# templeblock/llzlab

Hardware: AMD Instinct MI355X
Metric: Msamples/s/GPU (float32 FIR 257-tap, 4096 ch) + achieved HBM GB/s vs peak (higher is better)
Workload: dtype f32; 1 GPU; 4096-ch float32 FIR, 257 taps (llz_fir_lpf_cof 0.1 KAISER), 1048576 samples/ch per GPU, overlap-save-1024, channels sharded over 1 GPU(s); channels_per_gpu=4096, samples_per_channel=1048576, taps=257, algorithm=overlap-save-1024

## Files before the change

### llzlab_amd/csrc/kernels/fir_bank.hip

```cpp
#include "common.hpp"
#include "fft32.hpp"
#include "ols_walk.hpp"

namespace {

constexpr int BANK_BINS = LLZS_BANK_BINS;
constexpr int BANK_PITCH = LLZS_BANK_PITCH;
constexpr int BANK_IMG = 514;
constexpr size_t BANK_LDS_COMMON = 1024 * sizeof(float2) + (size_t)OLS_WAVES * 2 * OLS_XBUF * sizeof(float);

__device__ __forceinline__ void bank_filter(cf (&v)[32], cf (&u)[32], float *buf, const float2 *s_tw, const float2 *h, int l5,
                                            int col)
{
    ols_forward(v, buf, s_tw, l5, col);
    const float2 *up = h + l5, *dn = h - l5;
#pragma unroll
    for (int r = 0; r < 32; r++) {
        const int b = brev5(r);
        if (b < 16) {
            const float2 w = up[32 * b];
            u[b] = cmul<false>(v[r], cf{w.x, w.y});
        } else {
            const float2 w = dn[1024 - 32 * b];
            u[b] = cmul<true>(v[r], cf{w.x, w.y});
        }
    }
    ols_inverse(u, buf, s_tw, l5, col);
}

template <bool GLOBAL_H>
__global__ void __launch_bounds__(OLS_THREADS, 2)
k_fir_bank_ols_f32(const float *__restrict__ in, float *__restrict__ out, const float *__restrict__ hist,
                   const float2 *__restrict__ hbank , const float2 *__restrict__ twid, ols_geom G)
{
    extern __shared__ __attribute__((aligned(16))) char smem[];
    float2 *s_tw = reinterpret_cast<float2 *>(smem);
    for (int i = threadIdx.x; i < 1024; i += OLS_THREADS) s_tw[i] = twid[i];
    __syncthreads();
    const int lane = threadIdx.x & 63;
    const int wave = __builtin_amdgcn_readfirstlane(threadIdx.x >> 6);
    const int l5 = lane & 31;
    const ols_lane g = ols_lane_of(lane);
    const int slot = (threadIdx.x >> 6) * 2 + g.half;
    float *buf = reinterpret_cast<float *>(s_tw + 1024) + slot * OLS_XBUF;
    float2 *img = reinterpret_cast<float2 *>(smem + BANK_LDS_COMMON) + slot * BANK_IMG;
    const long halves_total = (long)gridDim.x * OLS_WAVES * 2;
    const long first = ((long)blockIdx.x * OLS_WAVES + wave) * 2;

    ols_seg cur[2] = {ols_locate(first, G), ols_locate(first + 1, G)};
    float halo[8];
    ols_raw raw;
    {
        const float *const row[2] = {in + (size_t)cur[0].c * G.in_pitch, in + (size_t)cur[1].c * G.in_pitch};
        const ols_seg own = g.half ? cur[1] : cur[0];
        ols_load_halo(halo, g.half ? row[1] : row[0], hist ? hist + (size_t)own.c * G.keep : nullptr, own.j0 * OLS_JOB,
                      g.col, G.keep, own.live);
        const int s0[2] = {cur[0].j0 * OLS_JOB, cur[1].j0 * OLS_JOB};
        const bool lv[2] = {cur[0].count > 0, cur[1].count > 0};
        ols_load(raw, row, s0, lv, g, G.n);
    }
    for (long sp = first; sp < G.total_segs; sp += halves_total) {
        const ols_seg nxt[2] = {ols_locate(sp + halves_total, G), ols_locate(sp + halves_total + 1, G)};
        const float *const row[2] = {in + (size_t)cur[0].c * G.in_pitch, in + (size_t)cur[1].c * G.in_pitch};
        float *const orow[2] = {out + (size_t)cur[0].c * G.out_pitch, out + (size_t)cur[1].c * G.out_pitch};
        const float *const nrow[2] = {in + (size_t)nxt[0].c * G.in_pitch, in + (size_t)nxt[1].c * G.in_pitch};
        const ols_seg nown = g.half ? nxt[1] : nxt[0];
        float halo_n[8];
#pragma unroll
        for (int i = 0; i < 8; i++) halo_n[i] = 0.f;

        const ols_seg own = g.half ? cur[1] : cur[0];
        const float2 *hrow = hbank + (size_t)own.c * BANK_PITCH;
        if (!GLOBAL_H && own.live) {
#pragma unroll
            for (int i = 0; i < 16; i++) img[l5 + 32 * i] = hrow[l5 + 32 * i];
            if (l5 == 0) img[BANK_BINS - 1] = hrow[BANK_BINS - 1];
        }
        const float2 *h = GLOBAL_H ? hrow : img;

        const int jmax = max(cur[0].count, cur[1].count);
#pragma unroll 1
        for (int jj = 0; jj < jmax; jj++) {
            const int s[2] = {(cur[0].j0 + jj) * OLS_JOB, (cur[1].j0 + jj) * OLS_JOB};
            const bool live[2] = {jj < cur[0].count, jj < cur[1].count};
            cf v[32], u[32];
            ols_assemble(v, halo, raw);
            const bool in_pair = jj + 1 < jmax;
            {
                const float *const lrow[2] = {in_pair ? row[0] : nrow[0], in_pair ? row[1] : nrow[1]};
                const int sn[2] = {in_pair ? s[0] + OLS_JOB : nxt[0].j0 * OLS_JOB,
                                   in_pair ? s[1] + OLS_JOB : nxt[1].j0 * OLS_JOB};
                const bool ln[2] = {in_pair ? jj + 1 < cur[0].count : nxt[0].count > 0,
                                    in_pair ? jj + 1 < cur[1].count : nxt[1].count > 0};
                ols_load(raw, lrow, sn, ln, g, G.n);
            }
            if (!in_pair)
                ols_load_halo(halo_n, g.half ? nrow[1] : nrow[0], hist ? hist + (size_t)nown.c * G.keep : nullptr,
                              nown.j0 * OLS_JOB, g.col, G.keep, nown.live);
            bank_filter(v, u, buf, s_tw, h, l5, g.col);
            ols_store(u, orow, s, live, g, G.n);
        }
        cur[0] = nxt[0];
        cur[1] = nxt[1];
#pragma unroll
        for (int i = 0; i < 8; i++) halo[i] = halo_n[i];
    }
}

const ols_rung BANK_RUNGS[2] = {
    {1024, 1, "k_fir_bank_ols_f32", OLS_THREADS, 2 * OLS_WAVES, 2, true, 1.0,
     BANK_LDS_COMMON + (size_t)OLS_WAVES * 2 * BANK_IMG * sizeof(float2), false, false,
     1, {OLS_HALO}, {kfn(k_fir_bank_ols_f32<false>)}},
    {1024, 1, "k_fir_bank_ols_f32<global>", OLS_THREADS, 2 * OLS_WAVES, 2, true, 1.0,
     BANK_LDS_COMMON, false, false,
     1, {OLS_HALO}, {kfn(k_fir_bank_ols_f32<true>)}},
};

}

extern "C" int llzs_fir_bank_ols_f32(const float *hbank, const float *twid, const float *in, float *out, const float *hist,
                                     int channels, int n, long in_pitch, long out_pitch, int flt_len, void *stream)
{
    if (!hbank || !twid || !in || !out || channels <= 0 || n <= 0 || in_pitch < n || out_pitch < n) {
        llzs_set_error("fir_bank_ols_f32: bad arguments");
        return LLZ_ERR_ARG;
    }
    if (flt_len < 1 || flt_len - 1 > OLS_HALO) {
        llzs_set_error("fir_bank_ols_f32: flt_len %d outside 1..%d", flt_len, OLS_HALO + 1);
        return LLZ_ERR_RANGE;
    }
    const ols_rung &r = BANK_RUNGS[llzs_tune(LLZS_TUNE_BANK_GLOBAL_H) == 1 ? 1 : 0];
    ols_plan p = ols_plan_of(r, channels, n, in_pitch, out_pitch, flt_len);
    const float2 *hf = reinterpret_cast<const float2 *>(hbank), *tw = reinterpret_cast<const float2 *>(twid);
    void *args[6] = {&in, &out, &hist, &hf, &tw, &p.G};
    const void *kernel = r.kernel[0];
    if (r.lds_bytes > 64 * 1024)
        LLZ_HIP_CHECK(hipFuncSetAttribute(kernel, hipFuncAttributeMaxDynamicSharedMemorySize, (int)r.lds_bytes));
    (void)hipLaunchKernel(kernel, dim3((unsigned)p.blocks), dim3(r.threads), args, r.lds_bytes, as_stream(stream));
    LLZ_LAUNCH_CHECK(r.name);
    return LLZ_OK;
}
```

### llzlab_amd/csrc/kernels/fir_ols.hip

```cpp
#include <stdlib.h>
#include "common.hpp"
#include "fft32.hpp"
#include "ols_walk.hpp"

namespace {

constexpr int OLS_OVERLAP = 256;
static_assert(OLS_OVERLAP == OLS_HALO, "ols_walk.hpp carries the same overlap");

struct ols_smem {
    float2 *tw, *h;
    float *buf;
};

__device__ __forceinline__ ols_smem ols_tables(char *smem, const float2 *__restrict__ hfreq, const float2 *__restrict__ twid)
{
    ols_smem m;
    m.tw = reinterpret_cast<float2 *>(smem);
    m.h = m.tw + 1024;
    for (int i = threadIdx.x; i < 1024; i += OLS_THREADS) {
        m.tw[i] = twid[i];
        m.h[i] = hfreq[i];
    }
    __syncthreads();
    const int wave = threadIdx.x >> 6, half = (threadIdx.x >> 5) & 1;
    m.buf = reinterpret_cast<float *>(m.h + 1024) + (wave * 2 + half) * OLS_XBUF;
    return m;
}

__global__ void __launch_bounds__(OLS_THREADS, 2)
k_fir_ols_chain_f32(const float *__restrict__ in, float *__restrict__ out, const float *__restrict__ hist,
                    const float2 *__restrict__ hfreq, const float2 *__restrict__ twid, ols_geom G)
{
    extern __shared__ __attribute__((aligned(16))) char smem[];
    const ols_smem S = ols_tables(smem, hfreq, twid);
    const int lane = threadIdx.x & 63;
    const int wave = __builtin_amdgcn_readfirstlane(threadIdx.x >> 6);
    const int l5 = lane & 31;
    const ols_lane g = ols_lane_of(lane);
    const long halves_total = (long)gridDim.x * OLS_WAVES * 2;
    const long first = ((long)blockIdx.x * OLS_WAVES + wave) * 2;

    ols_seg cur[2] = {ols_locate(first, G), ols_locate(first + 1, G)};
    float halo[8];
    ols_raw raw;
    {
        const float *const row[2] = {in + (size_t)cur[0].c * G.in_pitch, in + (size_t)cur[1].c * G.in_pitch};
        const ols_seg own = g.half ? cur[1] : cur[0];
        ols_load_halo(halo, g.half ? row[1] : row[0], hist ? hist + (size_t)own.c * G.keep : nullptr, own.j0 * OLS_JOB,
                      g.col, G.keep, own.live);
        const int s0[2] = {cur[0].j0 * OLS_JOB, cur[1].j0 * OLS_JOB};
        const bool lv[2] = {cur[0].count > 0, cur[1].count > 0};
        ols_load(raw, row, s0, lv, g, G.n);
    }
    for (long sp = first; sp < G.total_segs; sp += halves_total) {
        const ols_seg nxt[2] = {ols_locate(sp + halves_total, G), ols_locate(sp + halves_total + 1, G)};
        const float *const row[2] = {in + (size_t)cur[0].c * G.in_pitch, in + (size_t)cur[1].c * G.in_pitch};
        float *const orow[2] = {out + (size_t)cur[0].c * G.out_pitch, out + (size_t)cur[1].c * G.out_pitch};
        const float *const nrow[2] = {in + (size_t)nxt[0].c * G.in_pitch, in + (size_t)nxt[1].c * G.in_pitch};
        const ols_seg nown = g.half ? nxt[1] : nxt[0];
        float halo_n[8];
#pragma unroll
        for (int i = 0; i < 8; i++) halo_n[i] = 0.f;

        const int jmax = max(cur[0].count, cur[1].count);
#pragma unroll 1
        for (int jj = 0; jj < jmax; jj++) {
            const int s[2] = {(cur[0].j0 + jj) * OLS_JOB, (cur[1].j0 + jj) * OLS_JOB};
            const bool live[2] = {jj < cur[0].count, jj < cur[1].count};
            cf v[32], u[32];
            ols_assemble(v, halo, raw);
            const bool in_pair = jj + 1 < jmax;
            {
                const float *const lrow[2] = {in_pair ? row[0] : nrow[0], in_pair ? row[1] : nrow[1]};
                const int sn[2] = {in_pair ? s[0] + OLS_JOB : nxt[0].j0 * OLS_JOB,
                                   in_pair ? s[1] + OLS_JOB : nxt[1].j0 * OLS_JOB};
                const bool ln[2] = {in_pair ? jj + 1 < cur[0].count : nxt[0].count > 0,
                                    in_pair ? jj + 1 < cur[1].count : nxt[1].count > 0};
                ols_load(raw, lrow, sn, ln, g, G.n);
            }
            if (!in_pair)
                ols_load_halo(halo_n, g.half ? nrow[1] : nrow[0], hist ? hist + (size_t)nown.c * G.keep : nullptr,
                              nown.j0 * OLS_JOB, g.col, G.keep, nown.live);
            ols_filter(v, u, S.buf, S.tw, S.h, l5, g.col);
            ols_store(u, orow, s, live, g, G.n);
        }
        cur[0] = nxt[0];
        cur[1] = nxt[1];
#pragma unroll
        for (int i = 0; i < 8; i++) halo[i] = halo_n[i];
    }
}



template <int O>
__global__ void __launch_bounds__(OLS_THREADS, 2)
k_fir_ols2k_chain_f32(const float *__restrict__ in, float *__restrict__ out, const float *__restrict__ hist,
                     const float2 *__restrict__ hfreq2 ,
                     const float2 *__restrict__ twid , const float2 *__restrict__ tw2k ,
                     ols_geom G)
{
    extern __shared__ __attribute__((aligned(16))) char smem[];
    float2 *s_tw = reinterpret_cast<float2 *>(smem);
    float2 *s_h = s_tw + 1024;
    float2 *s_w = s_h + 2048;
    for (int i = threadIdx.x; i < 1024; i += OLS_THREADS) {
        s_tw[i] = twid[i];
        s_h[i] = hfreq2[i];
        s_h[1024 + i] = hfreq2[1024 + i];
        s_w[i] = tw2k[i];
    }
    __syncthreads();
    constexpr int O2K_OVERLAP = O, O2K_VALID = 2048 - O, O2K_JOB = 2 * O2K_VALID;
    constexpr int HP = O / 64, NEW = 32 - HP;
    const int lane = threadIdx.x & 63;
    const int wave = __builtin_amdgcn_readfirstlane(threadIdx.x >> 6);
    const int half = lane >> 5, l5 = lane & 31;
    float *buf = reinterpret_cast<float *>(s_w + 1024) + (wave * 2 + half) * OLS_XBUF;
    const float2 *my_h = s_h + half * 1024;
    const long waves_total = (long)gridDim.x * OLS_WAVES;
    const int rowoff = 32 * half + l5;

    struct segd { const float *row; float *orow; const float *hrow; int j0, count; };
    auto locate = [&](long seg) {
        segd d;
        const bool live = seg < G.total_segs;
        const int c = live ? (int)(seg / G.segs_per_channel) : 0;
        d.j0 = live ? (int)(seg - (long)c * G.segs_per_channel) * G.seg_len : 0;
        d.count = live ? min(G.seg_len, G.jobs_per_channel - d.j0) : 0;
        d.row = in + (size_t)c * G.in_pitch;
        d.orow = out + (size_t)c * G.out_pitch;
        d.hrow = hist ? hist + (size_t)c * G.keep : nullptr;
        return d;
    };
    const int n = G.n;
    auto load_halo = [&](float (&halo)[HP], const segd &d) {
#pragma unroll
        for (int i = 0; i < HP; i++) {
            const int idx = d.j0 * O2K_JOB - O2K_OVERLAP + 64 * i + rowoff;
            float v = 0.f;
            if (d.count > 0) {
                if (idx >= 0) v = d.row[idx];
                else if (d.hrow && idx >= -G.keep) v = d.hrow[G.keep + idx];
            }
            halo[i] = v;
        }
    };
    ols_raw raw;
    auto load = [&](const float *row, int s, bool live) {
        if (live && s + O2K_JOB <= n) {
#pragma unroll
            for (int i = 0; i < NEW; i++) {
                raw.a[i] = __builtin_nontemporal_load(&row[s + 64 * i + rowoff]);
                raw.b[i] = __builtin_nontemporal_load(&row[s + O2K_VALID + 64 * i + rowoff]);
            }
        } else {
#pragma unroll
            for (int i = 0; i < NEW; i++) {
                const int ia = s + 64 * i + rowoff, ib = ia + O2K_VALID;
                const float xa = row[min(ia, n - 1)], xb = row[min(ib, n - 1)];
                raw.a[i] = (live && ia < n) ? xa : 0.f;
                raw.b[i] = (live && ib < n) ? xb : 0.f;
            }
        }
    };

    long seg = (long)blockIdx.x * OLS_WAVES + wave;
    segd cur = locate(seg);
    float halo[HP];
    load_halo(halo, cur);
    load(cur.row, cur.j0 * O2K_JOB, cur.count > 0);
    for (; seg < G.total_segs; seg += waves_total) {
        const segd nxt = locate(seg + waves_total);
        float halo_n[HP];
#pragma unroll
        for (int i = 0; i < HP; i++) halo_n[i] = 0.f;
#pragma unroll 1
        for (int jj = 0; jj < cur.count; jj++) {
            const int s = (cur.j0 + jj) * O2K_JOB;
            const float *row = cur.row;
            float *orow = cur.orow;
            cf v[32], u[32];
#pragma unroll
            for (int i = 0; i < HP; i++) {
                v[i].x = halo[i];
                v[i].y = raw.a[NEW - HP + i];
                halo[i] = raw.b[NEW - HP + i];
            }
#pragma unroll
            for (int i = 0; i < NEW; i++) {
                v[HP + i].x = raw.a[i];
                v[HP + i].y = raw.b[i];
            }
            const bool in_seg = jj + 1 < cur.count;
            load(in_seg ? row : nxt.row, in_seg ? s + O2K_JOB : nxt.j0 * O2K_JOB, in_seg || nxt.count > 0);
            if (!in_seg) load_halo(halo_n, nxt);
            cf w[32];
#pragma unroll
            for (int p = 0; p < 16; p++) {
                cf sm = cadd(v[p], v[p + 16]);
                const float2 t = s_w[64 * p + rowoff];
                cf df = cmul<false>(csub(v[p], v[p + 16]), cf{t.x, t.y});
                swap32(sm.x, df.x);
                swap32(sm.y, df.y);
                w[2 * p] = sm;
                w[2 * p + 1] = df;
            }
            ols_filter(w, u, buf, s_tw, my_h, l5, l5);
            const bool whole = s + O2K_JOB <= n;
            const int oa = s - O2K_OVERLAP + rowoff, ob = oa + O2K_VALID;
#pragma unroll
            for (int p = 0; p < 16; p++) {
                cf P = u[brev5(2 * p)], Q = u[brev5(2 * p + 1)];
                swap32(P.x, Q.x);
                swap32(P.y, Q.y);
                const float2 t = s_w[64 * p + rowoff];
                Q = cmul<true>(Q, cf{t.x, t.y});
                const cf y0 = cadd(P, Q), y1 = csub(P, Q);
                if (whole) {
                    if (p >= HP) {
                        __builtin_nontemporal_store(y0.x, &orow[oa + 64 * p]);
                        __builtin_nontemporal_store(y0.y, &orow[ob + 64 * p]);
                    }
                    __builtin_nontemporal_store(y1.x, &orow[oa + 64 * (p + 16)]);
                    __builtin_nontemporal_store(y1.y, &orow[ob + 64 * (p + 16)]);
                } else {
                    if (p >= HP) {
                        if (oa + 64 * p < n) orow[oa + 64 * p] = y0.x;
                        if (ob + 64 * p < n) orow[ob + 64 * p] = y0.y;
                    }
                    if (oa + 64 * (p + 16) < n) orow[oa + 64 * (p + 16)] = y1.x;
                    if (ob + 64 * (p + 16) < n) orow[ob + 64 * (p + 16)] = y1.y;
                }
            }
        }
        cur = nxt;
#pragma unroll
        for (int i = 0; i < HP; i++) halo[i] = halo_n[i];
    }
}


__device__ __forceinline__ int o8k_lane()
{
    int l = (int)__builtin_amdgcn_mbcnt_hi(~0u, __builtin_amdgcn_mbcnt_lo(~0u, 0u));
    asm volatile("" : "+v"(l));
    return l;
}
constexpr int O4K_WAVES = 8, O4K_THREADS = 64 * O4K_WAVES;

template <int WS = 1>
__device__ __forceinline__ void ols2k_core(cf (&v)[32], cf (&y)[32], float *buf, const float2 *s_tw, const float2 *my_h,
                                           const float2 *s_w, int l5, int rowoff)
{
    cf w[32], u[32];
#pragma unroll
    for (int p = 0; p < 16; p++) {
        cf sm = cadd(v[p], v[p + 16]);
        const float2 t = s_w[WS * (64 * p + rowoff)];
        cf df = cmul<false>(csub(v[p], v[p + 16]), cf{t.x, t.y});
        swap32(sm.x, df.x);
        swap32(sm.y, df.y);
        w[2 * p] = sm;
        w[2 * p + 1] = df;
    }
    ols_filter(w, u, buf, s_tw, my_h, l5, l5);
#pragma unroll
    for (int p = 0; p < 16; p++) {
        cf P = u[brev5(2 * p)], Q = u[brev5(2 * p + 1)];
        swap32(P.x, Q.x);
        swap32(P.y, Q.y);
        const float2 t = s_w[WS * (64 * p + rowoff)];
        Q = cmul<true>(Q, cf{t.x, t.y});
        y[p] = cadd(P, Q);
        y[p + 16] = csub(P, Q);
    }
}

template <int O>
__global__ void __launch_bounds__(O4K_THREADS, 2)
k_fir_ols4k_f32(const float *__restrict__ in, float *__restrict__ out, const float *__restrict__ hist,
                const float2 *__restrict__ hfreq4 , const float2 *__restrict__ twid ,
                const float2 *__restrict__ tw2k , const float2 *__restrict__ tw4k ,
                ols_geom G)
{
    constexpr int V = 4096 - O, JOB = 2 * V, PO = O / 64, PV = V / 64;
    extern __shared__ __attribute__((aligned(16))) char smem[];
    float2 *s_tw = reinterpret_cast<float2 *>(smem);
    float2 *s_w2 = s_tw + 1024;
    float2 *s_w4 = s_w2 + 1024;
    float2 *s_h = s_w4 + 2048;
    for (int i = threadIdx.x; i < 1024; i += O4K_THREADS) {
        s_tw[i] = twid[i];
        s_w2[i] = tw2k[i];
        s_w4[i] = tw4k[i];
        s_w4[1024 + i] = tw4k[1024 + i];
#pragma unroll
        for (int j = 0; j < 4; j++) s_h[1024 * j + i] = hfreq4[1024 * j + i];
    }
    __syncthreads();
    const int wave = __builtin_amdgcn_readfirstlane(threadIdx.x >> 6);
    float *s_buf = reinterpret_cast<float *>(s_h + 4096);
    const long waves_total = (long)gridDim.x * O4K_WAVES;
    const int n = G.n;

    for (long seg = (long)blockIdx.x * O4K_WAVES + wave; seg < G.total_segs; seg += waves_total) {
        const int c = (int)(seg / G.segs_per_channel);
        const int j0 = (int)(seg - (long)c * G.segs_per_channel) * G.seg_len;
        const int count = min(G.seg_len, G.jobs_per_channel - j0);
        const float *row = in + (size_t)c * G.in_pitch;
        float *orow = out + (size_t)c * G.out_pitch;
        const float *hrow = hist ? hist + (size_t)c * G.keep : nullptr;
#pragma unroll 1
        for (int jj = 0; jj < count; jj++) {
            const int s = (j0 + jj) * JOB;
            cf v[64];
            const bool whole = s >= O && s + JOB <= n;
            {
            const int rowoff = o8k_lane();
            if (whole) {
#pragma unroll
                for (int i = 0; i < PO; i++) v[i].x = row[s - O + 64 * i + rowoff];
#pragma unroll
                for (int i = PO; i < 64; i++) v[i].x = __builtin_nontemporal_load(&row[s - O + 64 * i + rowoff]);
#pragma unroll
                for (int i = PO; i < 64; i++) v[i].y = __builtin_nontemporal_load(&row[s + V - O + 64 * i + rowoff]);
            } else {
#pragma unroll
                for (int i = 0; i < 64; i++) {
                    const int ia = s - O + 64 * i + rowoff;
                    float xa = 0.f;
                    if (ia >= 0) xa = row[min(ia, n - 1)];
                    else if (hrow && ia >= -G.keep) xa = hrow[G.keep + ia];
                    v[i].x = ia < n ? xa : 0.f;
                }
#pragma unroll
                for (int i = PO; i < 64; i++) {
                    const int ib = s + V - O + 64 * i + rowoff;
                    const float xb = row[min(ib, n - 1)];
                    v[i].y = ib < n ? xb : 0.f;
                }
            }
            }
#pragma unroll
            for (int i = 0; i < PO; i++) v[i].y = v[i + PV].x;
            const int rowoff = o8k_lane(), half = rowoff >> 5, l5 = rowoff & 31;
            float *buf = s_buf + (wave * 2 + half) * OLS_XBUF;
            cf e[32], o[32];
#pragma unroll
            for (int p = 0; p < 32; p++) {
                e[p] = cadd(v[p], v[p + 32]);
                const float2 t = s_w4[64 * p + rowoff];
                o[p] = cmul<false>(csub(v[p], v[p + 32]), cf{t.x, t.y});
            }
            cf ye[32], yo[32];
            ols2k_core(e, ye, buf, s_tw, s_h + (2 * half) * 1024, s_w2, l5, rowoff);
            ols2k_core(o, yo, buf, s_tw, s_h + (2 * half + 1) * 1024, s_w2, l5, rowoff);
            const bool all_out = s + JOB <= n;
#pragma unroll
            for (int p = 0; p < 32; p++) {
                if (p + 32 < PO) continue;
                const float2 t = s_w4[64 * p + rowoff];
                const cf q = cmul<true>(yo[p], cf{t.x, t.y});
                if (p >= PO) {
                    const cf y0 = cadd(ye[p], q);
                    const int oa = s + 64 * (p - PO) + rowoff, ob = oa + V;
                    if (all_out) {
                        __builtin_nontemporal_store(y0.x, &orow[oa]);
                        __builtin_nontemporal_store(y0.y, &orow[ob]);
                    } else {
                        if (oa < n) orow[oa] = y0.x;
                        if (ob < n) orow[ob] = y0.y;
                    }
                }
                const cf y1 = csub(ye[p], q);
                const int oa = s + 64 * (p + 32 - PO) + rowoff, ob = oa + V;
                if (all_out) {
                    __builtin_nontemporal_store(y1.x, &orow[oa]);
                    __builtin_nontemporal_store(y1.y, &orow[ob]);
                } else {
                    if (oa < n) orow[oa] = y1.x;
                    if (ob < n) orow[ob] = y1.y;
                }
            }
        }
    }
}


#ifdef O8K_TRACE
__device__ unsigned long long o8k_trace_buf[2048 * 8];
#define O8K_T0() unsigned long long o8_t = __builtin_readcyclecounter(), o8_acc[8] = {0, 0, 0, 0, 0, 0, 0, 0}
#define O8K_MARK(i) do { const unsigned long long now = __builtin_readcyclecounter(); o8_acc[i] += now - o8_t; o8_t = now; } while (0)
#define O8K_PIN(x) asm volatile("s_nop 0" ::"v"(x))
#define O8K_DUMP() do { if ((threadIdx.x & 63) == 0) { const unsigned wv_ = (blockIdx.x * (blockDim.x >> 6) + (threadIdx.x >> 6)) & 2047u; \
    for (int i = 0; i < 8; i++) o8k_trace_buf[wv_ * 8 + i] = o8_acc[i]; } } while (0)
#else
#define O8K_T0() do { } while (0)
#define O8K_MARK(i) do { } while (0)
#define O8K_PIN(x) do { } while (0)
#define O8K_DUMP() do { } while (0)
#endif
struct w128_tab {
    float c[64], s[64];
};
constexpr double o8k_sin(double x)
{
    double term = x, sum = x;
    for (int k = 1; k < 16; k++) {
        term *= -x * x / (double)((2 * k) * (2 * k + 1));
        sum += term;
    }
    return sum;
}
constexpr double o8k_cos(double x)
{
    double term = 1.0, sum = 1.0;
    for (int k = 1; k < 16; k++) {
        term *= -x * x / (double)((2 * k - 1) * (2 * k));
        sum += term;
    }
    return sum;
}
constexpr w128_tab o8k_make_w128()
{
    w128_tab t{};
    for (int j = 0; j < 64; j++) {
        const double a = 3.14159265358979323846 * (double)j / 64.0;
        t.c[j] = j == 32 ? 0.f : (float)o8k_cos(a);
        t.s[j] = j == 0 ? 0.f : (float)o8k_sin(a);
    }
    return t;
}
__device__ constexpr w128_tab kW128 = o8k_make_w128();

constexpr int O8K_WAVES = 8, O8K_THREADS = 64 * O8K_WAVES, O8K_PAIRS = O8K_WAVES / 2;
#ifndef O8K_SPIN
#define O8K_SPIN (1 << 18)
#endif
constexpr int O8K_SPIN_LIMIT = O8K_SPIN;

typedef __attribute__((address_space(3))) volatile int *o8k_flag_p;
typedef float o8k_f2 __attribute__((ext_vector_type(2)));
typedef __attribute__((address_space(3))) o8k_f2 *o8k_box_p;
struct o8k_pair {
    o8k_flag_p my_free, my_sent, pt_free, pt_sent;
    o8k_box_p my_box, pt_box;
    int k;
};
__device__ __forceinline__ void o8k_signal(o8k_flag_p flag, int k)
{
    asm volatile("s_waitcnt lgkmcnt(0)" ::: "memory");
    *flag = k;
}
__device__ __forceinline__ void o8k_wait(o8k_flag_p flag, int k)
{
    int spins = 0;
    while (__builtin_amdgcn_readfirstlane(*flag) < k && ++spins < O8K_SPIN_LIMIT) __builtin_amdgcn_s_sleep(1);
    asm volatile("" ::: "memory");
}
template <int OFF>
__device__ __forceinline__ void o8k_swap(cf (&a)[64], o8k_pair &ps)
{
    const int lane = o8k_lane();
    const o8k_box_p mine = ps.my_box + lane, theirs = ps.pt_box + lane;
#pragma unroll
    for (int r = 0; r < 2; r++) {
        ps.k++;
        o8k_signal(ps.my_free, ps.k);
        o8k_wait(ps.pt_free, ps.k);
#pragma unroll
        for (int i = 0; i < 16; i++) theirs[64 * i] = (o8k_f2){a[OFF + 16 * r + i].x, a[OFF + 16 * r + i].y};
        o8k_signal(ps.my_sent, ps.k);
        o8k_wait(ps.pt_sent, ps.k);
#pragma unroll
        for (int i = 0; i < 16; i++) {
            const o8k_f2 t = mine[64 * i];
            a[OFF + 16 * r + i] = cf{t[0], t[1]};
        }
    }
    asm volatile("s_waitcnt lgkmcnt(0)" ::: "memory");
}

__device__ __forceinline__ void ols4k_core(cf (&a)[64], float *buf, const float2 *s_tw, const float2 *s_w4, const float2 *h_e,
                                           const float2 *h_o, int l5, int rowoff)
{
    cf e[32], o[32];
#pragma unroll
    for (int p = 0; p < 32; p++) {
        e[p] = cadd(a[p], a[p + 32]);
        const float2 t = s_w4[64 * p + rowoff];
        o[p] = cmul<false>(csub(a[p], a[p + 32]), cf{t.x, t.y});
    }
    cf ye[32], yo[32];
    ols2k_core<2>(e, ye, buf, s_tw, h_e, s_w4, l5, rowoff);
    ols2k_core<2>(o, yo, buf, s_tw, h_o, s_w4, l5, rowoff);
#pragma unroll
    for (int p = 0; p < 32; p++) {
        const float2 t = s_w4[64 * p + rowoff];
        const cf q = cmul<true>(yo[p], cf{t.x, t.y});
        a[p] = cadd(ye[p], q);
        a[p + 32] = csub(ye[p], q);
    }
}

template <int O>
__global__ void __launch_bounds__(O8K_THREADS, 2)
k_fir_ols8k_f32(const float *__restrict__ in, float *__restrict__ out, const float *__restrict__ hist,
                const float2 *__restrict__ hfreq8 , const float2 *__restrict__ twid ,
                const float2 *__restrict__ tw4k , ols_geom G)
{
    constexpr int V = 8192 - O, JOB = 2 * V, PO = O / 64;
    static_assert(O % 64 == 0 && O <= 6144, "at least 2048 new samples per block");
    extern __shared__ __attribute__((aligned(16))) char smem[];
    float2 *s_tw = reinterpret_cast<float2 *>(smem);
    float2 *s_w4 = s_tw + 1024;
    float2 *s_h = s_w4 + 2048;
    float *s_buf = reinterpret_cast<float *>(s_h + 8192);
    int *s_flag = reinterpret_cast<int *>(s_buf + 2 * O8K_WAVES * OLS_XBUF);
    float2 *s_wl = reinterpret_cast<float2 *>(s_flag + 2 * O8K_WAVES);
    for (int i = threadIdx.x; i < 1024; i += O8K_THREADS) {
        s_tw[i] = twid[i];
        s_w4[i] = tw4k[i];
        s_w4[1024 + i] = tw4k[1024 + i];
#pragma unroll
        for (int j = 0; j < 8; j++) s_h[1024 * j + i] = hfreq8[1024 * j + i];
    }
    if (threadIdx.x < 2 * O8K_WAVES) s_flag[threadIdx.x] = 0;
    if (threadIdx.x < 64) {
        float sn, cs;
        sincospif((float)threadIdx.x * (1.0f / 4096.0f), &sn, &cs);
        s_wl[threadIdx.x] = make_float2(cs, -sn);
    }
    __syncthreads();
    const int wave = __builtin_amdgcn_readfirstlane(threadIdx.x >> 6);
#ifdef O8K_CROSS_SIMD
    const int w = wave & 1, pair = wave >> 1, partner = wave ^ 1;
#else
    const int w = wave >> 2, pair = wave & 3, partner = wave ^ 4;
#endif
    o8k_pair ps;
    ps.my_free = (o8k_flag_p)(s_flag + 2 * wave);
    ps.my_sent = (o8k_flag_p)(s_flag + 2 * wave + 1);
    ps.pt_free = (o8k_flag_p)(s_flag + 2 * partner);
    ps.pt_sent = (o8k_flag_p)(s_flag + 2 * partner + 1);
    ps.my_box = (o8k_box_p)(reinterpret_cast<o8k_f2 *>(s_buf + (wave * 2) * OLS_XBUF));
    ps.pt_box = (o8k_box_p)(reinterpret_cast<o8k_f2 *>(s_buf + (partner * 2) * OLS_XBUF));
    ps.k = 0;
    O8K_T0();
    const long pairs_total = (long)gridDim.x * O8K_PAIRS;
    const int n = G.n;
    const int pos0 = 32 * w;

    for (long seg = (long)blockIdx.x * O8K_PAIRS + pair; seg < G.total_segs; seg += pairs_total) {
        const int c = (int)(seg / G.segs_per_channel);
        const int j0 = (int)(seg - (long)c * G.segs_per_channel) * G.seg_len;
        const int count = min(G.seg_len, G.jobs_per_channel - j0);
        const float *row = in + (size_t)c * G.in_pitch;
        float *orow = out + (size_t)c * G.out_pitch;
        const float *hrow = hist ? hist + (size_t)c * G.keep : nullptr;
#pragma unroll 1
        for (int jj = 0; jj < count; jj++) {
            const int s = (j0 + jj) * JOB;
            O8K_MARK(6);
            cf a[64];
            const bool whole = s >= O && s + JOB <= n;
            if (whole) {
                const float *ra = row + s - O + 64 * pos0 + o8k_lane(), *rb = ra + V;
#pragma unroll
                for (int j = 0; j < 32; j++) {
                    a[j].x = __builtin_nontemporal_load(&ra[64 * j]);
                    a[32 + j].x = __builtin_nontemporal_load(&ra[64 * (j + 64)]);
                }
#pragma unroll
                for (int j = 0; j < 32; j++) {
                    a[j].y = __builtin_nontemporal_load(&rb[64 * j]);
                    a[32 + j].y = __builtin_nontemporal_load(&rb[64 * (j + 64)]);
                }
            } else {
                const int lane = o8k_lane();
#pragma unroll
                for (int j = 0; j < 64; j++) {
                    const int pos = pos0 + (j < 32 ? j : j + 32);
                    const int ia = s - O + 64 * pos + lane, ib = ia + V;
                    float xa = 0.f;
                    if (ia >= 0) xa = row[min(ia, n - 1)];
                    else if (hrow && ia >= -G.keep) xa = hrow[G.keep + ia];
                    a[j].x = ia < n ? xa : 0.f;
                    float xb;
                    if (O > 4096 && ib < 0) xb = (hrow && ib >= -G.keep) ? hrow[G.keep + ib] : 0.f;
                    else xb = row[min(ib, n - 1)];
                    a[j].y = ib < n ? xb : 0.f;
                }
            }
            O8K_PIN(a[0].x); O8K_PIN(a[63].y); O8K_PIN(a[31].y); O8K_PIN(a[32].x);
            O8K_MARK(0);
            const float2 wd = s_wl[o8k_lane()];
            const cf wv = w ? cf{wd.y, -wd.x} : cf{wd.x, wd.y};
#pragma unroll
            for (int j = 0; j < 32; j++) {
                const cf sm = cadd(a[j], a[32 + j]), df = csub(a[j], a[32 + j]);
                const cf t = cmul<false>(cf{kW128.c[j], -kW128.s[j]}, wv);
                const cf dt = cmul<false>(df, t);
                a[j] = w ? dt : sm;
                a[32 + j] = w ? sm : dt;
            }
            O8K_PIN(a[0].x); O8K_PIN(a[63].y);
            O8K_MARK(1);
            o8k_swap<32>(a, ps);
            O8K_PIN(a[32].x); O8K_PIN(a[63].y);
            O8K_MARK(2);
            {
                const int ln = o8k_lane(), hf = ln >> 5;
                ols4k_core(a, s_buf + (wave * 2 + hf) * OLS_XBUF, s_tw, s_w4, s_h + (4 * hf + w) * 1024, s_h + (4 * hf + 2 + w) * 1024,
                           ln & 31, ln);
            }
            O8K_PIN(a[0].x); O8K_PIN(a[63].y); O8K_PIN(a[32].x);
            O8K_MARK(3);
            if (w) {
                const float2 wr = s_wl[o8k_lane()];
                const cf wu = cf{wr.x, wr.y};
#pragma unroll
                for (int p = 0; p < 64; p++) {
                    const cf t = cmul<false>(cf{kW128.c[p ^ 32], -kW128.s[p ^ 32]}, wu);
                    a[p] = cmul<true>(a[p], t);
                }
            }
            o8k_swap<32>(a, ps);
            O8K_PIN(a[32].x); O8K_PIN(a[63].y); O8K_PIN(a[0].x);
            O8K_MARK(4);
            const float sg = w ? -1.f : 1.f;
            const int lane = o8k_lane();
            const bool all_out = s + JOB <= n;
            const int jmin = PO - pos0;
            float *oa0 = orow + s + 64 * (pos0 - PO) + lane;
#pragma unroll
            for (int j = 0; j < 32; j++) {
                const cf y0 = cadd(a[j], a[32 + j]), d1 = csub(a[j], a[32 + j]);
                const cf y1 = cf{d1.x * sg, d1.y * sg};
                const int oa = s + 64 * (pos0 + j - PO) + lane, ob = oa + V;
                if (all_out) {
                    if (j >= jmin) {
                        __builtin_nontemporal_store(y0.x, &oa0[64 * j]);
                        __builtin_nontemporal_store(y0.y, &oa0[64 * j + V]);
                    }
                    if (PO <= 64 || j >= jmin - 64) {
                        __builtin_nontemporal_store(y1.x, &oa0[64 * (j + 64)]);
                        __builtin_nontemporal_store(y1.y, &oa0[64 * (j + 64) + V]);
                    }
                } else {
                    if (j >= jmin) {
                        if (oa < n) orow[oa] = y0.x;
                        if (ob < n) orow[ob] = y0.y;
                    }
                    if (PO <= 64 || j >= jmin - 64) {
                        if (oa + 4096 < n) orow[oa + 4096] = y1.x;
                        if (ob + 4096 < n) orow[ob + 4096] = y1.y;
                    }
                }
            }
            O8K_MARK(5);
#ifdef O8K_TRACE
            o8_acc[7]++;
#endif
        }
    }
    O8K_DUMP();
}


const ols_rung OLS_RUNGS[] = {
    {1024, 1, "k_fir_ols_f32", OLS_THREADS, 2 * OLS_WAVES, 2, true, 1.0,
     2 * 1024 * sizeof(float2) + (size_t)OLS_WAVES * 2 * OLS_XBUF * sizeof(float), false, false,
     1, {OLS_OVERLAP}, {kfn(k_fir_ols_chain_f32)}},
    {2048, 2, "k_fir_ols2k_chain_f32", OLS_THREADS, OLS_WAVES, 2, false, 1.0,
     4 * 1024 * sizeof(float2) + (size_t)OLS_WAVES * 2 * OLS_XBUF * sizeof(float), true, false,
     2, {512, 1024}, {kfn(k_fir_ols2k_chain_f32<512>), kfn(k_fir_ols2k_chain_f32<1024>)}},
    {4096, 2, "k_fir_ols4k_f32", O4K_THREADS, O4K_WAVES, 1, false, 0.0,
     8 * 1024 * sizeof(float2) + (size_t)O4K_WAVES * 2 * OLS_XBUF * sizeof(float), true, true,
     7, {512, 768, 1024, 1536, 2048, 2560, 3072},
     {kfn(k_fir_ols4k_f32<512>), kfn(k_fir_ols4k_f32<768>), kfn(k_fir_ols4k_f32<1024>), kfn(k_fir_ols4k_f32<1536>),
      kfn(k_fir_ols4k_f32<2048>), kfn(k_fir_ols4k_f32<2560>), kfn(k_fir_ols4k_f32<3072>)}},
    {8192, 2, "k_fir_ols8k_f32", O8K_THREADS, O8K_PAIRS, 1, false, 0.0,
     (1024 + 2048 + 8192) * sizeof(float2) + (size_t)O8K_WAVES * 2 * OLS_XBUF * sizeof(float) + 2 * O8K_WAVES * sizeof(int) +
         64 * sizeof(float2), false, true,
     8, {1536, 2304, 2560, 3072, 3584, 4096, 5120, 6144},
     {kfn(k_fir_ols8k_f32<1536>), kfn(k_fir_ols8k_f32<2304>), kfn(k_fir_ols8k_f32<2560>), kfn(k_fir_ols8k_f32<3072>),
      kfn(k_fir_ols8k_f32<3584>), kfn(k_fir_ols8k_f32<4096>), kfn(k_fir_ols8k_f32<5120>), kfn(k_fir_ols8k_f32<6144>)}},
};

}

extern "C" int llzs_fir_ols_f32(int nfft, const llzs_ols_tables *t, const float *in, float *out, const float *hist, int channels,
                                int n, long in_pitch, long out_pitch, int flt_len, void *stream)
{
    const ols_rung *r = nullptr;
    for (const ols_rung &c : OLS_RUNGS)
        if (c.nfft == nfft) r = &c;
    if (!r || !t || !t->hfreq || !t->twid || (r->w2k && !t->tw2k) || (r->w4k && !t->tw4k) || !in || !out || channels <= 0 ||
        n <= 0 || in_pitch < n || out_pitch < n) {
        llzs_set_error("fir_ols_f32: bad arguments (%d points)", nfft);
        return LLZ_ERR_ARG;
    }
    if (flt_len < r->min_taps || flt_len - 1 > r->overlap[r->count - 1]) {
        llzs_set_error("fir_ols_f32: flt_len %d outside %d..%d (%d points)", flt_len, r->min_taps, r->overlap[r->count - 1] + 1,
                       nfft);
        return LLZ_ERR_RANGE;
    }
    ols_plan p = ols_plan_of(*r, channels, n, in_pitch, out_pitch, flt_len);
    const float2 *hf = reinterpret_cast<const float2 *>(t->hfreq), *tw = reinterpret_cast<const float2 *>(t->twid),
                 *w2 = reinterpret_cast<const float2 *>(t->tw2k), *w4 = reinterpret_cast<const float2 *>(t->tw4k);
    void *args[8] = {&in, &out, &hist, &hf, &tw};
    int k = 5;
    if (r->w2k) args[k++] = &w2;
    if (r->w4k) args[k++] = &w4;
    args[k] = &p.G;
    const void *kernel = r->kernel[p.instance];
    if (r->lds_bytes > 64 * 1024)
        LLZ_HIP_CHECK(hipFuncSetAttribute(kernel, hipFuncAttributeMaxDynamicSharedMemorySize, (int)r->lds_bytes));
    (void)hipLaunchKernel(kernel, dim3((unsigned)p.blocks), dim3(r->threads), args, r->lds_bytes, as_stream(stream));
    LLZ_LAUNCH_CHECK(r->name);
    return LLZ_OK;
}

#ifdef O8K_TRACE
extern "C" int llzs_o8k_trace_read(unsigned long long *dst, int count)
{
    LLZ_HIP_CHECK(hipDeviceSynchronize());
    LLZ_HIP_CHECK(hipMemcpyFromSymbol(dst, HIP_SYMBOL(o8k_trace_buf), sizeof(unsigned long long) * (size_t)count));
    return LLZ_OK;
}
#endif
```

### llzlab_amd/csrc/kernels/ols_walk.hpp

```cpp
#pragma once
#include "common.hpp"
#include "fft32.hpp"

namespace {

constexpr int OLS_N = 1024;
constexpr int OLS_HALO = 256;
constexpr int OLS_VALID = OLS_N - OLS_HALO;
constexpr int OLS_JOB = 2 * OLS_VALID;
constexpr int OLS_WAVES = 4;
constexpr int OLS_THREADS = 64 * OLS_WAVES;
constexpr int OLS_SEG = 16;

struct ols_lane {
    int half, col;
};

__device__ __forceinline__ ols_lane ols_lane_of(int lane)
{
    ols_lane g;
    g.half = lane >> 5;
    g.col = lane & 31;
    return g;
}

struct ols_seg {
    bool live;
    int c, j0, count;
};

struct ols_geom {
    int n, keep, jobs_per_channel, segs_per_channel, seg_len;
    long total_segs, in_pitch, out_pitch;
};

__device__ __forceinline__ ols_seg ols_locate(long seg, const ols_geom &G)
{
    ols_seg g;
    g.live = seg < G.total_segs;
    g.c = g.live ? (int)(seg / G.segs_per_channel) : 0;
    g.j0 = g.live ? (int)(seg - (long)g.c * G.segs_per_channel) * G.seg_len : 0;
    g.count = g.live ? min(G.seg_len, G.jobs_per_channel - g.j0) : 0;
    return g;
}

struct ols_raw {
    float a[24], b[24];
};

__device__ __forceinline__ void ols_load(ols_raw &raw, const float *const (&row)[2], const int (&s)[2],
                                         const bool (&live)[2], const ols_lane &g, int n)
{
    const bool whole = live[0] && live[1] && s[0] + OLS_JOB <= n && s[1] + OLS_JOB <= n;
    const float *r = g.half ? row[1] : row[0];
    const int so = g.half ? s[1] : s[0];
    const bool lv = g.half ? live[1] : live[0];
    if (whole) {
#pragma unroll
        for (int i = 0; i < 24; i++) {
            raw.a[i] = __builtin_nontemporal_load(&r[so + 32 * i + g.col]);
            raw.b[i] = __builtin_nontemporal_load(&r[so + OLS_VALID + 32 * i + g.col]);
        }
    } else {
#pragma unroll
        for (int i = 0; i < 24; i++) {
            const int ia = so + 32 * i + g.col, ib = ia + OLS_VALID;
            const float xa = r[min(ia, n - 1)], xb = r[min(ib, n - 1)];
            raw.a[i] = (lv && ia < n) ? xa : 0.f;
            raw.b[i] = (lv && ib < n) ? xb : 0.f;
        }
    }
}

__device__ __forceinline__ void ols_load_halo(float (&halo)[8], const float *row, const float *hrow, int s, int col,
                                              int keep, bool live)
{
#pragma unroll
    for (int i = 0; i < 8; i++) {
        const int idx = s - OLS_HALO + 32 * i + col;
        float v = 0.f;
        if (live) {
            if (idx >= 0) v = row[idx];
            else if (hrow && idx >= -keep) v = hrow[keep + idx];
        }
        halo[i] = v;
    }
}

__device__ __forceinline__ void ols_forward(cf (&v)[32], float *buf, const float2 *s_tw, int l5, int col)
{
    fft32<false>(v);
    transpose_twiddle<false>(v, buf, s_tw, col, l5);
    fft32<false>(v);
}

__device__ __forceinline__ void ols_inverse(cf (&u)[32], float *buf, const float2 *s_tw, int l5, int col)
{
    fft32<true>(u);
    transpose_twiddle<true>(u, buf, s_tw, l5, col);
    fft32<true>(u);
}

__device__ __forceinline__ void ols_filter(cf (&v)[32], cf (&u)[32], float *buf, const float2 *s_tw,
                                           const float2 *s_h, int l5, int col)
{
    ols_forward(v, buf, s_tw, l5, col);
#pragma unroll
    for (int r = 0; r < 32; r++) {
        const float2 h = s_h[l5 + 32 * brev5(r)];
        u[brev5(r)] = cmul<false>(v[r], cf{h.x, h.y});
    }
    ols_inverse(u, buf, s_tw, l5, col);
}

__device__ __forceinline__ void ols_store(const cf (&u)[32], float *const (&orow)[2], const int (&s)[2],
                                          const bool (&live)[2], const ols_lane &g, int n)
{
    const bool whole = live[0] && live[1] && s[0] + OLS_JOB <= n && s[1] + OLS_JOB <= n;
    const bool lv = g.half ? live[1] : live[0];
    if (!lv) return;
    float *o = g.half ? orow[1] : orow[0];
    const int so = g.half ? s[1] : s[0];
    const int oa = so + g.col - OLS_HALO;
    const int ob = oa + OLS_VALID;
    if (whole) {
#pragma unroll
        for (int r = 0; r < 32; r++) {
            const int n1 = brev5(r);
            if (n1 >= 8) {
                __builtin_nontemporal_store(u[r].x, &o[oa + 32 * n1]);
                __builtin_nontemporal_store(u[r].y, &o[ob + 32 * n1]);
            }
        }
    } else {
#pragma unroll
        for (int r = 0; r < 32; r++) {
            const int n1 = brev5(r);
            if (n1 >= 8) {
                if (oa + 32 * n1 < n) o[oa + 32 * n1] = u[r].x;
                if (ob + 32 * n1 < n) o[ob + 32 * n1] = u[r].y;
            }
        }
    }
}

__device__ __forceinline__ void ols_assemble(cf (&v)[32], float (&halo)[8], const ols_raw &raw)
{
#pragma unroll
    for (int i = 0; i < 8; i++) {
        v[i].x = halo[i];
        v[i].y = raw.a[16 + i];
        halo[i] = raw.b[16 + i];
    }
#pragma unroll
    for (int i = 0; i < 24; i++) {
        v[8 + i].x = raw.a[i];
        v[8 + i].y = raw.b[i];
    }
}


struct ols_rung {
    int nfft, min_taps;
    const char *name;
    int threads;
    int segs_per_wg;
    int wg_per_cu;
    bool tuned;
    double startup;
    size_t lds_bytes;
    bool w2k, w4k;
    int count;
    int overlap[8];
    const void *kernel[8];
};

template <typename K> static const void *kfn(K k) { return reinterpret_cast<const void *>(k); }

struct ols_plan {
    int instance;
    long blocks;
    ols_geom G;
};

static ols_plan ols_plan_of(const ols_rung &r, int channels, int n, long in_pitch, long out_pitch, int flt_len)
{
    ols_plan p;
    p.instance = 0;
    while (r.overlap[p.instance] < flt_len - 1) p.instance++;
    const int job = 2 * (r.nfft - r.overlap[p.instance]);
    ols_geom &G = p.G;
    G.n = n;
    G.keep = flt_len - 1;
    G.in_pitch = in_pitch;
    G.out_pitch = out_pitch;
    G.jobs_per_channel = (n + job - 1) / job;
    const int tuned_per_cu = r.tuned ? llzs_tune(LLZS_TUNE_OLS_WG_PER_CU) : -1;
    const long max_blocks = 256L * (tuned_per_cu > 0 ? tuned_per_cu : r.wg_per_cu);
    const long slots = max_blocks * r.segs_per_wg;
    int seg_len = OLS_SEG;
    if ((long)((G.jobs_per_channel + OLS_SEG - 1) / OLS_SEG) * channels < 4 * slots) {
        double best = 1e300;
        for (int sl = OLS_SEG; sl >= 1; sl--) {
            const long segs = (long)((G.jobs_per_channel + sl - 1) / sl) * channels;
            const double cost = (double)((segs + slots - 1) / slots) * (sl + r.startup);
            if (cost < best * 0.999) { best = cost; seg_len = sl; }
        }
    }
    if (r.tuned)
        if (const int v = llzs_tune(LLZS_TUNE_OLS_SEG_LEN); v >= 1 && v <= 1024) seg_len = v;
    G.seg_len = seg_len;
    G.segs_per_channel = (G.jobs_per_channel + seg_len - 1) / seg_len;
    G.total_segs = (long)G.segs_per_channel * channels;
    p.blocks = (G.total_segs + r.segs_per_wg - 1) / r.segs_per_wg;
    if (p.blocks > max_blocks) p.blocks = max_blocks;
    return p;
}

}
```

Baseline: 646,000 Msamples/s.

## Add steady-state OLS loop with inline-asm prefetch and partial vmcnt waits

Adds a steady-state inner loop for full interior jobs in both the OLS and bank FIR kernels. It issues the next job's 48 loads as inline-asm nontemporal global_load_dword with immediate offsets, and waits with s_waitcnt vmcnt(48) so stores need not drain before the loads land. Stores use a simplified whole-job path with no bounds checks. The intent is to cut per-job address arithmetic and branch overhead and to overlap loads with the FFT. The risk is fragile hand-tuned wait counts, register pinning that constrains the compiler, and a generic loop still needed for the tail jobs.

Result: slower. 633,300 Msamples/s (-2.0%).

```diff
diff --git a/llzlab_amd/csrc/kernels/fir_bank.hip b/llzlab_amd/csrc/kernels/fir_bank.hip
--- a/llzlab_amd/csrc/kernels/fir_bank.hip
+++ b/llzlab_amd/csrc/kernels/fir_bank.hip
@@ -79,8 +79,12 @@
         const float2 *h = GLOBAL_H ? hrow : img;
 
         const int jmax = max(cur[0].count, cur[1].count);
+        const int jsteady = GLOBAL_H ? 0 : max(ols_steady_jobs(cur, G.n), 0);
+        if (jsteady > 0)
+            ols_steady(raw, halo, row, orow, cur, g, jsteady,
+                       [&](cf (&v)[32], cf (&u)[32]) { bank_filter(v, u, buf, s_tw, h, l5, g.col); });
 #pragma unroll 1
-        for (int jj = 0; jj < jmax; jj++) {
+        for (int jj = jsteady; jj < jmax; jj++) {
             const int s[2] = {(cur[0].j0 + jj) * OLS_JOB, (cur[1].j0 + jj) * OLS_JOB};
             const bool live[2] = {jj < cur[0].count, jj < cur[1].count};
             cf v[32], u[32];
diff --git a/llzlab_amd/csrc/kernels/fir_ols.hip b/llzlab_amd/csrc/kernels/fir_ols.hip
--- a/llzlab_amd/csrc/kernels/fir_ols.hip
+++ b/llzlab_amd/csrc/kernels/fir_ols.hip
@@ -64,8 +64,12 @@
         for (int i = 0; i < 8; i++) halo_n[i] = 0.f;
 
         const int jmax = max(cur[0].count, cur[1].count);
+        const int jsteady = max(ols_steady_jobs(cur, G.n), 0);
+        if (jsteady > 0)
+            ols_steady(raw, halo, row, orow, cur, g, jsteady,
+                       [&](cf (&v)[32], cf (&u)[32]) { ols_filter(v, u, S.buf, S.tw, S.h, l5, g.col); });
 #pragma unroll 1
-        for (int jj = 0; jj < jmax; jj++) {
+        for (int jj = jsteady; jj < jmax; jj++) {
             const int s[2] = {(cur[0].j0 + jj) * OLS_JOB, (cur[1].j0 + jj) * OLS_JOB};
             const bool live[2] = {jj < cur[0].count, jj < cur[1].count};
             cf v[32], u[32];
diff --git a/llzlab_amd/csrc/kernels/ols_walk.hpp b/llzlab_amd/csrc/kernels/ols_walk.hpp
--- a/llzlab_amd/csrc/kernels/ols_walk.hpp
+++ b/llzlab_amd/csrc/kernels/ols_walk.hpp
@@ -156,6 +156,96 @@
     for (int i = 0; i < 24; i++) {
         v[8 + i].x = raw.a[i];
         v[8 + i].y = raw.b[i];
+    }
+}
+
+
+#define OLS_LD_(k, off) "global_load_dword %" #k ", %12, off offset:" #off " nt\n\t"
+#define OLS_LD6_(a0, a1, a2, a3, a4, a5, b0, b1, b2, b3, b4, b5)                                                            \
+    OLS_LD_(0, a0) OLS_LD_(1, b0) OLS_LD_(2, a1) OLS_LD_(3, b1) OLS_LD_(4, a2) OLS_LD_(5, b2)                               \
+    OLS_LD_(6, a3) OLS_LD_(7, b3) OLS_LD_(8, a4) OLS_LD_(9, b4) OLS_LD_(10, a5) OLS_LD_(11, b5)
+#define OLS_OUT6_(r, i)                                                                                                      \
+    "=&v"(r.a[i]), "=&v"(r.b[i]), "=&v"(r.a[i + 1]), "=&v"(r.b[i + 1]), "=&v"(r.a[i + 2]), "=&v"(r.b[i + 2]),               \
+    "=&v"(r.a[i + 3]), "=&v"(r.b[i + 3]), "=&v"(r.a[i + 4]), "=&v"(r.b[i + 4]), "=&v"(r.a[i + 5]), "=&v"(r.b[i + 5])
+#define OLS_PIN6_(r, i)                                                                                                      \
+    "+v"(r.a[i]), "+v"(r.b[i]), "+v"(r.a[i + 1]), "+v"(r.b[i + 1]), "+v"(r.a[i + 2]), "+v"(r.b[i + 2]),                     \
+    "+v"(r.a[i + 3]), "+v"(r.b[i + 3]), "+v"(r.a[i + 4]), "+v"(r.b[i + 4]), "+v"(r.a[i + 5]), "+v"(r.b[i + 5])
+
+__device__ __forceinline__ void ols_request(ols_raw &raw, const float *mid)
+{
+    static_assert(OLS_VALID * sizeof(float) == 3072, "the literal offsets below");
+    asm volatile(OLS_LD6_(-3072, -2944, -2816, -2688, -2560, -2432, 0, 128, 256, 384, 512, 640)
+                 : OLS_OUT6_(raw, 0) : "v"(mid) : "memory");
+    asm volatile(OLS_LD6_(-2304, -2176, -2048, -1920, -1792, -1664, 768, 896, 1024, 1152, 1280, 1408)
+                 : OLS_OUT6_(raw, 6) : "v"(mid) : "memory");
+    asm volatile(OLS_LD6_(-1536, -1408, -1280, -1152, -1024, -896, 1536, 1664, 1792, 1920, 2048, 2176)
+                 : OLS_OUT6_(raw, 12) : "v"(mid) : "memory");
+    asm volatile(OLS_LD6_(-768, -640, -512, -384, -256, -128, 2304, 2432, 2560, 2688, 2816, 2944)
+                 : OLS_OUT6_(raw, 18) : "v"(mid) : "memory");
+}
+
+__device__ __forceinline__ void ols_pin(ols_raw &raw)
+{
+    asm volatile("" : OLS_PIN6_(raw, 0) : : "memory");
+    asm volatile("" : OLS_PIN6_(raw, 6) : : "memory");
+    asm volatile("" : OLS_PIN6_(raw, 12) : : "memory");
+    asm volatile("" : OLS_PIN6_(raw, 18) : : "memory");
+}
+
+__device__ __forceinline__ void ols_settle(ols_raw &raw, float (&halo)[8])
+{
+    asm volatile("s_waitcnt vmcnt(0)" ::: "memory");
+    ols_pin(raw);
+    asm volatile("" : "+v"(halo[0]), "+v"(halo[1]), "+v"(halo[2]), "+v"(halo[3]), "+v"(halo[4]), "+v"(halo[5]), "+v"(halo[6]),
+                      "+v"(halo[7]) : : "memory");
+}
+
+__device__ __forceinline__ void ols_await(ols_raw &raw)
+{
+    asm volatile("s_waitcnt vmcnt(48)" ::: "memory");
+    ols_pin(raw);
+}
+#undef OLS_LD_
+#undef OLS_LD6_
+#undef OLS_OUT6_
+#undef OLS_PIN6_
+
+__device__ __forceinline__ void ols_store_whole(const cf (&u)[32], float *dst)
+{
+#pragma unroll
+    for (int r = 0; r < 32; r++) {
+        const int n1 = brev5(r);
+        if (n1 >= 8) {
+            __builtin_nontemporal_store(u[r].x, &dst[32 * (n1 - 8)]);
+            __builtin_nontemporal_store(u[r].y, &dst[OLS_VALID + 32 * (n1 - 8)]);
+        }
+    }
+}
+
+__device__ __forceinline__ int ols_steady_jobs(const ols_seg (&cur)[2], int n)
+{
+    const int whole = n / OLS_JOB;
+    return min(min(cur[0].count, whole - cur[0].j0), min(cur[1].count, whole - cur[1].j0)) - 1;
+}
+
+template <typename F>
+__device__ __forceinline__ void ols_steady(ols_raw &raw, float (&halo)[8], const float *const (&row)[2], float *const (&orow)[2],
+                                           const ols_seg (&cur)[2], const ols_lane &g, int count, F &&filter)
+{
+    const int s0 = (g.half ? cur[1].j0 : cur[0].j0) * OLS_JOB + g.col;
+    const float *mid = (g.half ? row[1] : row[0]) + s0 + OLS_JOB + OLS_VALID;
+    float *dst = (g.half ? orow[1] : orow[0]) + s0;
+    ols_settle(raw, halo);
+#pragma unroll 1
+    for (int jj = 0; jj < count; jj++) {
+        cf v[32], u[32];
+        ols_assemble(v, halo, raw);
+        ols_request(raw, mid);
+        filter(v, u);
+        ols_store_whole(u, dst);
+        ols_await(raw);
+        mid += OLS_JOB;
+        dst += OLS_JOB;
     }
 }
 
```
